# aitor-martinez-seras/SNN-Automotive-Object-Detection

Measured on AMD Instinct MI355X. Metric: images/sec (T_rpn=8,T_det=12, 1024x2048 b=2) spiking RPN+RoI heads forward, higher is better.
Workload: dtype f32 (weights as exact bf16x3 split, fp32 accumulate); 1 GPU; cityscapes_1024x2048_b2_heads: RPNHeadSNN(T=8) on 5-level pyramid 2x256x{192x384..12x24} + FastRCNNPredictorSNNFull(T=12) on 2000 RoIs x 12544, K=9; random-init weights; inputs: FPN output of the random-init ResNet-50-FPN on seeded rand(3,1024,2048) images (transform 768/1536); RoI features = 7x7 RoIAlign of 1000 seeded boxes per image; precision=bf16x3, global_batch=2, parallelism=dp1, exchange=none

## Files before the change

### snn_automotive_object_detection_amd/csrc/snn_kernels.hip

```cpp
#include "snn_common.h"
#include "snn_hip.h"
#include "snn_hip_debug.h"

#if !defined(SNN_EXPERIMENTS) && (defined(SNN_EXP_NO_FETCH) || defined(SNN_EXP_NO_GLDS) || defined(SNN_EXP_NO_BARRIER) || \
    defined(SNN_EXP_CLOCK) || defined(SNN_EXP_TIMELINE) || defined(SNN_EXP_SP_NO_A) || defined(SNN_EXP_SP_NO_B) || defined(SNN_EXP_SP_NO_AREAD) || defined(SNN_EXP_SP_NO_BREAD) || defined(SNN_EXP_SP_NO_MFMA) || defined(SNN_EXP_SP_NO_BAR) || defined(SNN_EXP_ONE_WG_PER_CU) || defined(SNN_EXP_MX_NOSTAGE) || defined(SNN_EXP_MX_NOREADB) || defined(SNN_EXP_MX_NOBAR) || \
    defined(SNN_EXP_MX_NOA) || defined(SNN_EXP_MX_BAR2) || defined(SNN_EXP_MX_RDW_G) || defined(SNN_EXP_ENCP_NOLOAD) || defined(SNN_EXP_ENCP_NOENC) || defined(SNN_EXP_ENCP_NOSTORE) || \
    defined(SNN_EXP_PP_NOWAIT) || defined(SNN_EXP_PP_NOCOPY) || defined(SNN_EXP_PP_NOBAR) || defined(SNN_EXP_PP_NOMFMA) || defined(SNN_EXP_PP_NOEPI) || defined(SNN_EXP_PP_NOY) || defined(SNN_EXP_PP_ALLDENSE) || defined(SNN_EXP_PP_ALLSPARSE) || defined(SNN_EXP_PP_NOBREAD) || defined(SNN_EXP_SP_NO_SEC))
#error "SNN_EXP_* switches are timing experiments with wrong results: add -DSNN_EXPERIMENTS (never in a product build)"
#endif

#include <stdarg.h>
#include <stdio.h>
#include <stdlib.h>
#include <string.h>

static thread_local char g_err[512] = "";
static thread_local int g_last_fc_sparse = 0;
static thread_local unsigned long long g_last_rpn_planes[3] = {0, 0, 0};
static thread_local unsigned long long g_last_det_planes[3] = {0, 0, 0};
static thread_local int g_last_enc_mode = -1;
static thread_local int g_last_conv_sparse = 0;

static int fail(int code, const char* fmt, ...) __attribute__((format(printf, 2, 3)));
static int fail(int code, const char* fmt, ...) {
// ... 85 lines not shown
        }
        dst[idx] = v;
    }
}

#include "snn_encode.h"
#include "snn_f32.h"
#include "snn_bf16x3.h"
#include "snn_sparse.h"
#ifdef SNN_PINGPONG
#include "snn_sparse_pp.h"
#endif
#include "snn_heads.h"
#include "snn_post.h"

#include "snn_mx.h"

#include "snn_affine.h"
#include "snn_taps.h"
#include "snn_wgrad.h"
#include "snn_loss.h"
#include "snn_hidden.h"
#include "snn_spike_wgrad_x3.h"

#define SNN_SPARSE_FAT_CONV_DEFAULT 3
#ifndef SNN_CONV_PP_DEFAULT
#define SNN_CONV_PP_DEFAULT 0
#endif
struct Knobs {
    bool enc_generic;
    bool enc_rows_ballot;
    int bf16x3_mt;
    int bf16x3_short;
    int bf16x3_wn;
    bool bf16x3_lif_reg;
    int mx_mw;
    int li_heads;
    bool debug_occ;
    bool spk_rows;
    bool bf16x3_xcd;
    bool stage_wm;
    bool enc_quant;
    bool periods;
    bool stage_periods;
    int roi_e, roi_rw;
    bool epi_general;
    bool roi_tab;
    bool dead_keep;
    bool sparse;
    int encp_nw;
    int encp_rb;
    int sparse_fat_conv;
    bool lif_regs;
    bool conv_pp;
    bool enc_fold;
    bool sparse_fat;
    int planes;
};
static Knobs load_knobs() {
    Knobs k;
    const char* e;
    k.enc_generic = (e = getenv("SNN_ENC_GENERIC")) && e[0] == '1';
    k.enc_rows_ballot = (e = getenv("SNN_ENC_ROWS")) && !strcmp(e, "ballot");
    k.bf16x3_mt = (e = getenv("SNN_BF16X3_MT")) ? atoi(e) : 0;
    e = getenv("SNN_BF16X3_SHORT");
    k.bf16x3_short = (e && e[0] == '1') ? 1 : (e && e[0] == '0') ? 0 : -1;
    e = getenv("SNN_BF16X3_WN");
    k.bf16x3_wn = (e && e[0] == '2') ? 2 : (e && e[0] == '1') ? 1 : 0;
    k.bf16x3_lif_reg = (e = getenv("SNN_BF16X3_LIF")) && !strcmp(e, "reg");
    e = getenv("SNN_MX_MW");
    k.mx_mw = (e && e[0] == '8') ? 8 : ((e && e[0] == '4') ? 4 : 0);
    e = getenv("SNN_LI_HEADS");
    k.li_heads = !e ? 0 : !strcmp(e, "valu") ? 1 : !strcmp(e, "mfma") ? 2 : !strcmp(e, "ksplit") ? 3 : 4;
    k.debug_occ = getenv("SNN_DEBUG_OCC") != nullptr;
    k.sparse_fat = !((e = getenv("SNN_SPARSE_FAT")) && e[0] == '0');
    k.enc_fold = !((e = getenv("SNN_ENC_FOLD")) && e[0] == '0');
    k.conv_pp = (e = getenv("SNN_CONV_PP")) ? e[0] == '1' : SNN_CONV_PP_DEFAULT != 0;
    k.lif_regs = !((e = getenv("SNN_LIF_REGS")) && e[0] == '0');
    k.sparse_fat_conv = (e = getenv("SNN_SPARSE_FAT_CONV")) ? atoi(e) : SNN_SPARSE_FAT_CONV_DEFAULT;
    k.encp_rb = (e = getenv("SNN_ENCP_RB")) ? atoi(e) : 0;
    k.encp_nw = (e = getenv("SNN_ENCP_NW")) ? atoi(e) : 0;
    e = getenv("SNN_PLANES");
    k.planes = !e ? 0 : !strcmp(e, "rm") ? 1 : !strcmp(e, "wm") ? 2 : 0;
    k.bf16x3_xcd = !((e = getenv("SNN_BF16X3_XCD")) && e[0] == '0');
    k.spk_rows = (e = getenv("SNN_SPK_SPLIT")) && e[0] == '0';
    k.stage_wm = (e = getenv("SNN_STAGE_PLANES")) && !strcmp(e, "wm");
    k.dead_keep = (e = getenv("SNN_DEAD_STEPS")) && !strcmp(e, "keep");
    k.periods = !((e = getenv("SNN_PERIOD_PLANES")) && e[0] == '0');
    k.enc_quant = !((e = getenv("SNN_ENC_QUANT")) && e[0] == '0');
    k.stage_periods = (e = getenv("SNN_STAGE_PERIODS")) && e[0] == '1';
    k.epi_general = (e = getenv("SNN_EPI_GENERAL")) && e[0] == '1';
    k.roi_tab = !((e = getenv("SNN_ROI_TAB")) && e[0] == '0');
    k.sparse = !((e = getenv("SNN_SPARSE")) && e[0] == '0');
    k.roi_e = (e = getenv("SNN_ROI_E")) ? atoi(e) : 0;
    k.roi_rw = (e = getenv("SNN_ROI_RW")) ? atoi(e) : 0;
    if (k.roi_e < 0 || k.roi_e > 16) k.roi_e = 0;
    if (k.roi_rw < 0 || k.roi_rw > 8) k.roi_rw = 0;
    return k;
}
// ... 92 lines not shown
    const int force = knobs().bf16x3_mt;
    if (force == 8 && knobs().bf16x3_wn == 2 && tiles_of(8) > 0) return 8;
    for (int mt = 4; mt >= 2; --mt) {
        const long long wgs = tiles_of(mt);
        if (wgs <= 0) continue;
        if (force == mt) return mt;
        const double cost = (double)((wgs + g3_slots() - 1) / g3_slots()) * (mt + 0.5);
        if (best_cost == 0 || cost < best_cost * 0.97) { best = mt; best_cost = cost; }
    }
    return best;
}

struct G3Tile { int mt, n_short, rows; };
template <typename F>
static G3Tile g3_pick_tile(int wn, F wgs_of) {
    G3Tile best = {0, 0, 0};
    double best_cost = 0;
    const int force_mt = knobs().bf16x3_mt, force_short = knobs().bf16x3_short;
    const int nwm = 8 / wn;
    if (force_mt == 8 && knobs().bf16x3_wn == 2 && wgs_of(256) > 0) return G3Tile{8, 0, 256};
    for (int mt = 4; mt >= 2; --mt)
        for (int sh = 0; sh < 2; ++sh) {
            if (force_mt >= 2 && force_mt <= 4 && force_mt != mt) continue;
            if (force_short >= 0 && force_short != sh) continue;
            const int n_short = sh ? nwm / 2 : 0, rows = nwm * 16 * mt - 16 * n_short;
            const long long wgs = wgs_of(rows);
            if (wgs <= 0) continue;
            const double cost = (double)((wgs + g3_slots() - 1) / g3_slots()) * (mt - 0.5 * sh + 0.5);
            if (best_cost == 0 || cost < best_cost * 0.97) { best = G3Tile{mt, n_short, rows}; best_cost = cost; }
        }
    return best;
}

#ifndef G3_NB1
#define G3_NB1 4
#endif
static int g3_wn(bool conv = false) { (void)conv; return knobs().bf16x3_wn ? knobs().bf16x3_wn : 1; }

static int g3_bm(int wn, int mt) { return mt == 8 ? 256 : G3_BM(wn, mt); }

template <int MODE>
static const void* g3_kernel(int mt, int wn, int planes) {
    if (planes == 1) {
        if (wn == 2)
            return mt == 8 ? (const void*)k_gemm_bf16<MODE, 3, 8, 2>
                 : mt == 4 ? (const void*)k_gemm_bf16<MODE, 3, 4, 2> : mt == 3 ? (const void*)k_gemm_bf16<MODE, 3, 3, 2>
                                                                                : (const void*)k_gemm_bf16<MODE, 3, 2, 2>;
        return mt == 4 ? (const void*)k_gemm_bf16<MODE, G3_NB1, 4, 1> : mt == 3 ? (const void*)k_gemm_bf16<MODE, G3_NB1, 3, 1>
                                                                                  : (const void*)k_gemm_bf16<MODE, G3_NB1, 2, 1>;
    }
    if (wn == 2)
        return mt == 8 ? (const void*)k_gemm_bf16x3<MODE, 3, 8, 2>
             : mt == 4 ? (const void*)k_gemm_bf16x3<MODE, 3, 4, 2> : mt == 3 ? (const void*)k_gemm_bf16x3<MODE, 3, 3, 2>
                                                                              : (const void*)k_gemm_bf16x3<MODE, 3, 2, 2>;
    return mt == 4 ? (const void*)k_gemm_bf16x3<MODE, G3_NB1, 4, 1> : mt == 3 ? (const void*)k_gemm_bf16x3<MODE, G3_NB1, 3, 1>
                                                                                : (const void*)k_gemm_bf16x3<MODE, G3_NB1, 2, 1>;
}

__device__ __forceinline__ unsigned long long det_payload_key(const float* __restrict__ l, int K, int r) {
    float m = l[0];
    for (int c = 1; c < K; ++c) m = fmaxf(m, l[c]);
    float sum = 0.0f, best = -1.0f;
    int lab = 1;
    for (int c = 0; c < K; ++c) {
        const float e = expf(l[c] - m);
        sum += e;
        if (c >= 1 && e > best) { best = e; lab = c; }
    }
    const float score = best / sum;
    return ((unsigned long long)__float_as_uint(score) << 32) | ((unsigned long long)(0xFFFFu - (unsigned)r) << 16) | (unsigned)lab;
}

template <int E>
__global__ __launch_bounds__(1024) void k_det_payload(const float* __restrict__ cls, const float* __restrict__ reg, int Rn,
                                                      int K, int max_det, int npad, float* __restrict__ payload,
                                                      int* __restrict__ counts) {
    extern __shared__ __attribute__((aligned(16))) unsigned char smem[];
    unsigned long long* const keys = reinterpret_cast<unsigned long long*>(smem);
    const int img = blockIdx.x, tid = threadIdx.x, nthr = blockDim.x;
    const size_t base = (size_t)img * Rn;
    if (E == 1) {
        unsigned long long key = tid < Rn ? det_payload_key(cls + (base + tid) * K, K, tid) : 0ull;
        for (int k = 2; k <= npad; k <<= 1)
            for (int j = k >> 1; j > 0; j >>= 1) {
                unsigned long long other;
                if (j < 64) {
                    other = __shfl_xor(key, j);
                } else {
                    __syncthreads();
                    keys[tid] = key;
                    __syncthreads();
                    other = keys[tid ^ j];
                }
                const bool desc = (tid & k) == 0, lower = (tid & j) == 0;
                const bool take_max = desc == lower;
                key = take_max ? (key > other ? key : other) : (key < other ? key : other);
            }
        __syncthreads();
        keys[tid] = key;
        __syncthreads();
    } else {
        for (int r = tid; r < npad; r += nthr) keys[r] = r < Rn ? det_payload_key(cls + (base + r) * K, K, r) : 0ull;
        __syncthreads();
        for (int k = 2; k <= npad; k <<= 1)
            for (int j = k >> 1; j > 0; j >>= 1) {
                for (int i = tid; i < npad; i += nthr) {
                    const int ixj = i ^ j;
                    if (ixj > i) {
                        const unsigned long long a = keys[i], b = keys[ixj];
                        if ((i & k) == 0 ? a < b : a > b) { keys[i] = b; keys[ixj] = a; }
                    }
                }
                __syncthreads();
            }
    }
    const int n = min(max_det, Rn);
    for (int t = tid; t < max_det; t += nthr) {
        float* out = payload + ((size_t)img * max_det + t) * 6;
        if (t < n) {
            const unsigned long long key = keys[t];
            const int r = 0xFFFF - (int)((key >> 16) & 0xFFFFu), lab = (int)(key & 0xFFFFu);
            const float* d = reg + (base + r) * 4 * K + 4 * lab;
            out[0] = d[0]; out[1] = d[1]; out[2] = d[2]; out[3] = d[3];
            out[4] = __uint_as_float((uint32_t)(key >> 32));
            out[5] = (float)lab;
        } else {
            for (int q = 0; q < 6; ++q) out[q] = 0.0f;
        }
    }
    if (tid == 0) counts[img] = n;
}

#define ENC_PICKER(fn, K, KN)                                                                                                                              \
    template <int EM>                                                                                                                                      \
    static const void* fn##_of(int fdt) {                                                                                                                  \
        if (fdt & SNN_FEAT_NHWC) return KN<EM>(fdt & ~SNN_FEAT_NHWC);                                                                                      \
        return fdt == SNN_FEAT_F16 ? (const void*)K##_h<EM, feat_f16> : fdt == SNN_FEAT_BF16 ? (const void*)K##_h<EM, feat_bf16> : (const void*)K<EM>;      \
    }                                                                                                                                                      \
    static const void* fn(int em, int fdt) { return em == ENC_QUANT ? fn##_of<ENC_QUANT>(fdt) : em == ENC_ZR ? fn##_of<ENC_ZR>(fdt) : fn##_of<ENC_GENERIC>(fdt); }
template <int EM> static const void* enc_nhwc_stage(int dt) {
    return dt == SNN_FEAT_F16 ? (const void*)k_encode_nhwc<EM, feat_f16> : dt == SNN_FEAT_BF16 ? (const void*)k_encode_nhwc<EM, feat_bf16> : (const void*)k_encode_nhwc<EM, float>;
}
template <int EM> static const void* enc_nhwc_levels(int dt) {
    return dt == SNN_FEAT_F16 ? (const void*)k_encode_levels_nhwc<EM, feat_f16> : dt == SNN_FEAT_BF16 ? (const void*)k_encode_levels_nhwc<EM, feat_bf16>
                                                                                                       : (const void*)k_encode_levels_nhwc<EM, float>;
}
template <int EM> static const void* enc_nhwc_none(int) { return nullptr; }
ENC_PICKER(encode_nchw_kernel, k_encode_nchw, enc_nhwc_stage)
ENC_PICKER(encode_levels_kernel, k_encode_levels, enc_nhwc_levels)
ENC_PICKER(encode_rows_wm_kernel, k_encode_rows_wm, enc_nhwc_none)
#undef ENC_PICKER
static size_t feat_elem_bytes(int fdt) { return (fdt & ~SNN_FEAT_NHWC) == SNN_FEAT_F32 ? 4 : 2; }
template <int RB, int NW>
// ... 269 lines not shown
                                  snn_stream_t s) {
    if (!a_rows || !w_packed || !cur || M <= 0 || K <= 0 || N <= 0 || ldo < N)
        return fail(-1, "snn_spike_gemm_bf16x3: bad argument");
    Gemm3Args a;
    memset(&a, 0, sizeof(a));
    if ((long long)M * cdiv(K, 32) * 4 > 0xffffffffLL) return fail(-1, "snn_spike_gemm_bf16x3: spike rows over 4 GB");
    a.A = a_rows; a.wpk = w_packed; a.out = cur; a.M = M; a.Kc = cdiv(K, 32); a.Np = cdiv(N, 32) * 32; a.ldo = ldo;
    a.plane_elems = (unsigned long long)a.Kc * a.Np * 32;
    const int wn = g3_wn();
    a.n_blocks = cdiv(a.Np, G3_BN(wn));
    const int mt = g3_pick_mt([&](int m) { return (long long)cdiv(M, g3_bm(wn, m)) * a.n_blocks; });
    return launch_gemm3(G3_FC, mt, wn, a, planes, (hipStream_t)s);
}

int snn_spike_gemm_bf16x3(const uint32_t* a_rows, int M, int K, int N, const uint16_t* w_packed, float* cur, int ldo,
                          snn_stream_t s) {
    return spike_gemm_bf16x3_impl(a_rows, M, K, N, w_packed, cur, ldo, 3, s);
}

static int set_periods(Gemm3Args& a, const char* who) {
    if (a.t0 != 0) return fail(-1, "%s: period planes need a window that starts at step 0", who);
    a.periods = 1;
    for (int t = 0; t < SNN_MAX_STEPS; ++t) {
        a.div[t] = 0;
        if (t < a.Tc)
            for (int n = 1; n <= a.Tc; ++n)
                if ((t + 1) % n == 0) a.div[t] |= 1u << (n - 1);
    }
    return 0;
}

static int spike_gemm_lif_bf16x3_args(const uint32_t* a_planes, int T, int R, int K, int N, const snn_params* p,
                                      const uint16_t* w_packed, uint32_t* spk, size_t spk_stride, uint32_t* row_counts,
                                      bool wm_in, bool wm_out, const StepWindow* win, bool periods, Gemm3Args* out, G3Tile* tile) {
    if (!a_planes || !w_packed || !spk || !p || R <= 0 || K <= 0 || N <= 0)
        return fail(-1, "snn_spike_gemm_lif_bf16x3: bad argument");
    if (check_T(T, "snn_spike_gemm_lif_bf16x3")) return -1;
    if ((long long)T * R * cdiv(K, 32) * 4 > 0xffffffffLL) return fail(-1, "snn_spike_gemm_lif_bf16x3: input planes over 4 GB");
    Gemm3Args& a = *out;
    memset(&a, 0, sizeof(a));
    a.A = a_planes; a.wpk = w_packed; a.M = R; a.Kc = cdiv(K, 32); a.Np = cdiv(N, 32) * 32;
    a.plane_elems = (unsigned long long)a.Kc * a.Np * 32;
    const int wn = g3_wn();
    a.n_blocks = cdiv(a.Np, G3_BN(wn));
    a.T = T; a.spk = spk; a.spk_stride = spk_stride; a.p = make_p(p, p->v_th_lif); a.cnt_row = row_counts;
    a.wm = wm_in; a.out_wm = wm_out; a.a_step = (unsigned long long)R;
    const StepWindow w = win ? *win : lif_window_full_out(T);
    a.t0 = w.t0; a.Tc = w.n;
    const int Tc = w.n;
    const G3Tile tl = g3_pick_tile(wn, [&](int rows) { return g3_tile_ok(Tc, rows) ? (long long)cdiv(R, rows / Tc) * a.n_blocks : 0ll; });
    if (!tl.mt) return fail(-4, "snn_spike_gemm_lif_bf16x3: T=%d does not fit a row tile (use snn_spike_gemm_bf16x3 + snn_lif_scan)", T);
    a.pb = tl.rows / Tc; a.n_short = tl.n_short;
    if (periods && set_periods(a, "snn_spike_gemm_lif_bf16x3")) return -1;
    *tile = tl;
    return 0;
}

static int spike_gemm_lif_bf16x3_impl(const uint32_t* a_planes, int T, int R, int K, int N, const snn_params* p,
                                      const uint16_t* w_packed, uint32_t* spk, size_t spk_stride, uint32_t* row_counts, snn_stream_t s,
                                      bool wm_in = false, bool wm_out = false, const StepWindow* win = nullptr, bool periods = false) {
    Gemm3Args a;
    G3Tile tl;
    const int rc = spike_gemm_lif_bf16x3_args(a_planes, T, R, K, N, p, w_packed, spk, spk_stride, row_counts, wm_in, wm_out, win, periods, &a, &tl);
    if (rc) return rc;
    return launch_gemm3(G3_FC_LIF_TILE, tl.mt, g3_wn(), a, 3, (hipStream_t)s);
}

int snn_spike_gemm_lif_bf16x3(const uint32_t* a_planes, int T, int R, int K, int N, const snn_params* p,
                              const uint16_t* w_packed, uint32_t* spk, size_t spk_stride, snn_stream_t s) {
    return spike_gemm_lif_bf16x3_impl(a_planes, T, R, K, N, p, w_packed, spk, spk_stride, nullptr, s, knobs().stage_wm, false, nullptr,
                                      knobs().stage_periods);
}

static bool mx_tile_ok(int T) { return g3_tile_ok(T, MX_BM); }

static int mx_mw() { return knobs().mx_mw ? knobs().mx_mw : MX_MW_DEFAULT; }

#define MX_KERNEL_OF(MW, mode)                                                                        \
    ((mode) == G3_FC ? (const void*)k_gemm_mx<G3_FC, MW>                                              \
     : (mode) == G3_CONV ? (const void*)k_gemm_mx<G3_CONV, MW>                                        \
     : (mode) == G3_CONV_LIF_TILE ? (const void*)k_gemm_mx<G3_CONV_LIF_TILE, MW>                      \
                                  : (const void*)k_gemm_mx<G3_FC_LIF_TILE, MW>)

// ... 360 lines not shown
    SNN_CHECK_LAUNCH("k_gemm_lif_sparse");
    }
    if (cnt_pos) {
        PosCountArgs pa;
        memset(&pa, 0, sizeof(pa));
        pa.cnt_pos = cnt_pos; pa.cnt_img = a.cnt_img; pa.n_levels = a.n_levels; pa.max_n = a.max_n;
        memcpy(pa.lv, a.lv, sizeof(pa.lv));
        hipLaunchKernelGGL(k_sum_pos_counts, dim3(a.n_levels * a.max_n, POSCNT_CHUNKS), dim3(256), 0, s, pa);
        SNN_CHECK_LAUNCH("k_sum_pos_counts");
    }
    return gated ? 2 : 1;
}

int snn_debug_tile_shape(int conv, long long units, int k_in, int n_cols, int num_steps, int spike_rates, int layer, int32_t* out) {
    if (!out || units <= 0 || k_in <= 0 || n_cols <= 0 || num_steps < 1 || num_steps > SNN_MAX_STEPS) return fail(-1, "snn_debug_tile_shape: bad argument");
    snn_params p;
    memset(&p, 0, sizeof(p));
    p.v_th_lif = 0.1f;
    int Tc;
    if (conv) Tc = lif_window_full_out(num_steps).n;
    else { const DetWindows w = det_windows(&p, num_steps, spike_rates != 0); Tc = layer == 7 ? w.fc7.n : w.fc6.n; }
    memset(out, 0, 12 * sizeof(int32_t));
    SparseShape sh;
    const int Kw = cdiv(k_in, 32), Np = cdiv(n_cols, 32) * 32;
    if (knobs().periods && (conv || layer != 7) && sparse_shape(conv != 0, units, Kw, conv ? 9 * Kw : Kw, Np, num_steps, Tc, SPARSE_ROUTE, &sh)) {
        const SparsePlan& sp = sh.sp;
        int slots = 0;
        for (int w = 0; w < (sp.fat ? 4 : 8) / sp.wn; ++w) slots += sp.w_nd[w] + sp.w_ns[w];
        out[0] = sp.fat ? (sp.wn == 1 ? SP_MT_FAT : conv ? SP_MT2_FAT_CONV : SP_MT2_FAT) : sp.wn == 1 ? SP_MT : SP_MT2; out[1] = sp.fat; out[2] = Tc * sp.pb; out[3] = sp.pb; out[4] = Tc; out[5] = sh.n_tiles * sh.n_blocks;
        out[6] = sh.n_blocks; out[7] = sp.wn; out[8] = 1; out[9] = sp.nd; out[10] = Tc - sp.nd; out[11] = slots;
        return 0;
    }
    const int wn = g3_wn(conv != 0), n_blocks = cdiv(Np, G3_BN(wn));
    const G3Tile tl = g3_pick_tile(wn, [&](int rows) { return g3_tile_ok(Tc, rows) ? (long long)cdiv(units, rows / Tc) * n_blocks : 0ll; });
    if (!tl.mt) return fail(-4, "snn_debug_tile_shape: %d steps do not fit a row tile", num_steps);
    const int pb = tl.rows / Tc;
    out[0] = tl.mt; out[1] = tl.n_short; out[2] = tl.rows; out[3] = pb; out[4] = Tc; out[5] = (int32_t)(cdiv(units, pb) * n_blocks);
    out[6] = n_blocks; out[7] = wn; out[8] = 0; out[9] = Tc; out[10] = 0; out[11] = 0;
    return 0;
}

struct ConvLifOpts {
    bool wm = false;
    bool* out_split = nullptr;
    bool periods = false;
    void* sparse_side = nullptr;
    size_t sparse_bytes = 0;
    int sparse_mode = SPARSE_RUN;
    SparseRoute route = SPARSE_ROUTE;
    int planes = 3;
};
static int conv3x3_lif_bf16x3_impl(const uint32_t* enc, size_t enc_stride, const snn_rpn_level* lv, int n_levels, int C_in,
                                   int C_out, int T, const snn_params* p, const uint16_t* w_packed, uint32_t* spk,
                                   size_t spk_stride, unsigned long long* counts, int max_n, snn_stream_t s, const ConvLifOpts& o) {
    const bool wm = o.wm, periods = o.periods;
    const int sparse_mode = o.sparse_mode;
    const bool want_split = o.out_split && *o.out_split;
    if (o.out_split) *o.out_split = false;
    if (!spk || !p) return fail(-1, "snn_conv3x3_lif_bf16x3: bad argument");
    Gemm3Args a;
    long long P;
    int rc = conv3_common("snn_conv3x3_lif_bf16x3", enc, enc_stride, lv, n_levels, C_in, C_out, T, w_packed, a, &P);
    if (rc) return rc;
    if (wm) {
        if (enc_stride % a.Cw) return fail(-1, "snn_conv3x3_lif_bf16x3: word-major planes need enc_stride %% Cw == 0");
        a.wm = 1; a.a_step = enc_stride / a.Cw;
        if (a.a_step * (unsigned long long)a.Cw > 0x7fffffffULL) return fail(-1, "snn_conv3x3_lif_bf16x3: plane too large");
// ... 1164 lines not shown
static DetCall det_call(int fdt, int R, int Hd, int K, int K4, int T, const snn_params* p, const void* w6_packed, int w6_inner,
                        const void* w7_packed, const float* w_heads_packed, float* out_cls, float* out_bbox, uint32_t* spk6_count,
                        uint32_t* spk7_count, float* sum_cls, float* sum_bbox, void* ws, size_t ws_bytes, snn_stream_t stream) {
    DetCall c = {};
    c.fdt = fdt; c.R = R; c.Hd = Hd; c.K = K; c.K4 = K4; c.T = T; c.p = p;
    c.w6_packed = w6_packed; c.w6_inner = w6_inner; c.w7_packed = w7_packed; c.w_heads_packed = w_heads_packed;
    c.out_cls = out_cls; c.out_bbox = out_bbox; c.spk6_count = spk6_count; c.spk7_count = spk7_count; c.sum_cls = sum_cls; c.sum_bbox = sum_bbox;
    c.ws = ws; c.ws_bytes = ws_bytes; c.stream = stream;
    c.route = SPARSE_ROUTE;
    return c;
}
static void feed_rows(DetCall& c, const void* x, int D) { c.roi_fed = false; c.x = x; c.D = D; c.who = "snn_det_head_forward"; }
static void feed_roialign(DetCall& c, const snn_roi_level* levels_host, int n_levels, int C, const float* rois, const int* roi_batch,
                          const int* roi_level) {
    c.roi_fed = true; c.levels_host = levels_host; c.n_levels = n_levels; c.C = C; c.rois = rois; c.roi_batch = roi_batch; c.roi_level = roi_level;
    c.who = "snn_det_head_forward_roialign";
}

static int det_readouts_check(const char* who, const int* steps, int n, const uint32_t* c6, const uint32_t* c7, const float* sum_cls,
                              const float* sum_bbox) {
    if (check_steps(steps, n, who)) return -1;
    if ((c6 == nullptr) != (c7 == nullptr)) return fail(-1, "%s: spk6_count and spk7_count go together", who);
    if ((sum_cls == nullptr) != (sum_bbox == nullptr)) return fail(-1, "%s: sum_cls and sum_bbox go together", who);
    return 0;
}

struct DetPlan {
    size_t o_enc, o_cur, o_s6, o_s7;
    size_t o_raw;
    DetWindows win;
    bool wm, per;
    bool bin_major;
    bool gated;
};

static void det_planes_views(const DetPlan& dp, int R, int Hd, int T, snn_planes_view* v6, snn_planes_view* v7) {
    const int Hw = cdiv(Hd, 32);
    for (int i = 0; i < 2; ++i) {
        snn_planes_view* v = i ? v7 : v6;
        if (!v) continue;
        const StepWindow& w = i ? dp.win.fc7 : dp.win.fc6;
        v->offset_bytes = i ? dp.o_s7 : dp.o_s6; v->step_stride_words = (uint64_t)R * Hw; v->rows = R; v->words = Hw;
        v->layout = (!i && dp.wm) ? SNN_PLANES_WORD_MAJOR : SNN_PLANES_ROWS;
        v->steps_formed = min(T, w.t0 + w.n + 1);
        v->reserved = 0;
    }
}

static bool det_fc6_sparse_plan(const DetCall& c, int D, const DetPlan& dp) {
    Gemm3Args a6;
    G3Tile t6;
    return spike_gemm_lif_bf16x3_args((const uint32_t*)((char*)c.ws + dp.o_enc), c.T, c.R, D, c.Hd, c.p, (const uint16_t*)c.w6_packed,
                                      (uint32_t*)((char*)c.ws + dp.o_s6), (size_t)c.R * cdiv(c.Hd, 32), c.spk6_count, true, true, &dp.win.fc6, true,
                                      &a6, &t6) == 0 &&
           gemm3_lif_sparse(a6, false, (char*)c.ws + dp.o_cur, dp.o_s6 - dp.o_cur, (hipStream_t)c.stream, SPARSE_QUERY, c.route, weight_planes(c.p)) == 1;
}

static int det_plan(const DetCall& c, int D, bool wm_ok, DetPlan* dp) {
    size_t need;
    det_ws_layout(c.R, D, c.Hd, c.T, &dp->o_enc, &dp->o_cur, &dp->o_s6, &dp->o_s7, &need);
    if (c.ws_bytes < need) return fail(-2, "%s: workspace %zu < %zu bytes", c.who, c.ws_bytes, need);
    if (check_T(c.T, c.who)) return -1;
    dp->o_raw = c.w6_inner > 1 ? det_ws_perm_offset(c.R, D, c.Hd, c.T) : dp->o_enc;
    dp->bin_major = false;
    dp->win = det_windows(c.p, c.T, c.spk6_count != nullptr);
    dp->wm = det_planes_wm(c.p, dp->win) && wm_ok;
    dp->per = knobs().periods && periods_possible(c.p) && det_b3_tiles(c.p, dp->win);
    dp->gated = c.route.route == SNN_ROUTE_AUTO && c.route.stat && !c.spk6_count && !c.steps && c.w6_inner == 49 && dp->wm && dp->per &&
                det_fc6_sparse_plan(c, D, *dp);
    return 0;
}

static bool det_fc6_folds(bool feed_ok, const DetCall& c, int D, const DetPlan& dp, NeuronP* np, const EncTh** eth) {
    if (dp.gated || !knobs().enc_fold || !feed_ok || c.w6_inner != 49 || !dp.wm || !dp.per) return false;
    *np = make_p(c.p, c.p->v_th_enc);
    np->v_fire = ENC_FIRED;
    if (!enc_zero_rest(*np) || enc_mode(*np, eth) != ENC_QUANT) return false;
    return det_fc6_sparse_plan(c, D, dp);
}

static int det_heads_tail(const DetCall& c, const uint32_t* s6, const uint32_t* s7, bool s6_wm) {
    const int R = c.R, Hw = cdiv(c.Hd, 32);
    if (!c.steps)
        return snn_li_heads(s7, (size_t)R * Hw, c.T, R, c.Hd, c.w_heads_packed, c.K, c.K4, c.p, c.out_cls, c.out_bbox, c.sum_cls, c.sum_bbox, c.stream);
    int rc = li_heads_readouts_impl(s7, (size_t)R * Hw, c.steps, c.n_steps, R, c.Hd, c.w_heads_packed, c.K, c.K4, c.p, c.out_cls, c.out_bbox, c.sum_cls,
                                    c.sum_bbox, false, c.stream);
    if (rc || !c.spk6_count) return rc;
    const StepList st = step_list(c.steps, c.n_steps);
    hipLaunchKernelGGL(k_count_rows_ro, dim3(cdiv(R, 256)), dim3(256), 0, (hipStream_t)c.stream, s6, (unsigned long long)R * Hw, R, Hw, s6_wm ? 1 : 0, st, c.spk6_count);
    SNN_CHECK_LAUNCH("k_count_rows_ro");
    hipLaunchKernelGGL(k_count_rows_ro, dim3(cdiv(R, 256)), dim3(256), 0, (hipStream_t)c.stream, s7, (unsigned long long)R * Hw, R, Hw, 0, st, c.spk7_count);
    SNN_CHECK_LAUNCH("k_count_rows_ro");
    return 0;
}

static int fc6_route_fixed(int32_t* route_stat, int route_taken, hipStream_t s) {
    if (!route_stat) return 0;
// ... 22 lines not shown
    const int Hw = cdiv(Hd, 32), Hp = Hw * 32;
    snn_planes_view v6, v7;
    det_planes_views(dp, R, Hd, T, &v6, &v7);
    g_last_det_planes[0] = v6.offset_bytes; g_last_det_planes[1] = v7.offset_bytes; g_last_det_planes[2] = v6.layout == SNN_PLANES_WORD_MAJOR ? 1 : 0;
    int rc;
    if (k_inner > 1 && !folded && !dp.bin_major) {
        const int C = D / k_inner;
        if (D % k_inner || C % 32 || !enc_wm || !det_b3_tiles(p, win))
            return fail(-4, "snn_det_head_forward: permuted fc6 weights (inner = %d) need D = C * inner, C %% 32 == 0 and the fused bf16x3 path", k_inner);
        const uint32_t* enc_raw = (const uint32_t*)((char*)ws + dp.o_raw);
        const int Dw = cdiv(D, 32);
        if (k_inner != 49) return fail(-4, "snn_det_head_forward: permuted fc6 weights: inner = %d (only 49 = 7 x 7 bins is built)", k_inner);
        hipLaunchKernelGGL(k_permute_planes<49>, dim3(cdiv(R, 32), win.enc_steps), dim3(256), 0, s, enc_raw, enc, Dw, R, C);
        SNN_CHECK_LAUNCH("k_permute_planes");
    }
    if (spk6_count) { if (hipMemsetAsync(spk6_count, 0, sizeof(uint32_t) * R, s) != hipSuccess) return fail(-3, "hipMemsetAsync failed"); }
    if (spk7_count) { if (hipMemsetAsync(spk7_count, 0, sizeof(uint32_t) * R, s) != hipSuccess) return fail(-3, "hipMemsetAsync failed"); }
    const bool b3 = prec_family(p) == SNN_PRECISION_BF16X3, mx = prec_family(p) == SNN_PRECISION_MXFP6;
    if (prec_family(p) != SNN_PRECISION_F32 && !b3 && !mx) return fail(-1, "snn_det_head_forward: unknown precision %d", p->precision);
    if (mx) {
        if (D % 128 || Hd % 128)
            return fail(-4, "snn_det_head_forward: the mxfp6 kernels need D, Hd %% 128 == 0");
        if (!mx_tile_ok(win.fc6.n) || !mx_tile_ok(win.fc7.n)) return fail(-4, "snn_det_head_forward: T=%d does not fit a 512-row tile of the mxfp6 kernels", T);
        if ((rc = fc6_route_fixed(rt.stat, spk6_count ? 0 : 1, s))) return rc;
        if ((rc = spike_gemm_lif_mx_impl(enc, T, R, D, Hd, p, (const uint32_t*)w6_packed, s6, (size_t)R * Hw, spk6_count, stream, &win.fc6))) return rc;
        if ((rc = spike_gemm_lif_mx_impl(s6, T, R, Hd, Hd, p, (const uint32_t*)w7_packed, s7, (size_t)R * Hw, spk7_count, stream, &win.fc7))) return rc;
        return det_heads_tail(c, s6, s7, false);
    }
    if ((enc_wm || enc_periods) && !det_b3_tiles(p, win)) return fail(-1, "snn_det_head_forward: word-major / period planes without the fused bf16x3 layers");
    if (det_b3_tiles(p, win)) {
        Gemm3Args a6, a7;
        G3Tile t6, t7;
        if ((rc = spike_gemm_lif_bf16x3_args(enc, T, R, D, Hd, p, (const uint16_t*)w6_packed, s6, (size_t)R * Hw, spk6_count, enc_wm, enc_wm, &win.fc6, enc_periods, &a6, &t6))) return rc;
        if ((rc = spike_gemm_lif_bf16x3_args(s6, T, R, Hd, Hd, p, (const uint16_t*)w7_packed, s7, (size_t)R * Hw, spk7_count, enc_wm, false, &win.fc7, false, &a7, &t7))) return rc;
        const int wn = g3_wn();
        rc = gemm3_lif_sparse(a6, false, (char*)ws + o_cur, o_s6 - o_cur, s, folded ? SPARSE_RUN_COMPRESSED : SPARSE_RUN, rt, planes);
        if (rc < 0) return rc;
        if (folded && rc != 1) return fail(-3, "snn_det_head_forward: the encoder wrote compressed planes but fc6 takes the dense launch (internal)");
        if (rt.gated && rc != 2) return fail(-3, "snn_det_head_forward: fc6 route: the gated pair was planned but fc6 did not enqueue it (internal)");
        g_last_fc_sparse = rc;
        if (rc == 2) { a6.gate = (const int*)rt.stat + 2; a6.gate_want = 1; }
        else if ((rc = fc6_route_fixed(rt.stat, (spk6_count || rc == 1) ? 0 : 1, s))) return rc;
        if (g_last_fc_sparse != 1 && (rc = launch_gemm3(G3_FC_LIF_TILE, t6.mt, wn, a6, planes, s))) return rc;
        if ((rc = launch_gemm3(G3_FC_LIF_TILE, t7.mt, wn, a7, planes, s))) return rc;
        return det_heads_tail(c, s6, s7, enc_wm);
    }
    if ((rc = fc6_route_fixed(rt.stat, spk6_count ? 0 : 1, s))) return rc;
    const uint32_t* a6 = enc + (size_t)win.fc6.t0 * R * cdiv(D, 32);
    rc = b3 ? spike_gemm_bf16x3_impl(a6, win.fc6.n * R, D, Hd, (const uint16_t*)w6_packed, cur, Hp, planes, stream)
            : snn_spike_gemm(a6, win.fc6.n * R, D, Hd, (const float*)w6_packed, cur, Hp, stream);
    if (rc) return rc;
    if ((rc = lif_scan_window(cur, T, win.fc6, R, Hd, Hp, p, s6, (size_t)R * Hw, spk6_count, stream))) return rc;
    const uint32_t* a7 = s6 + (size_t)win.fc7.t0 * R * Hw;
    rc = b3 ? spike_gemm_bf16x3_impl(a7, win.fc7.n * R, Hd, Hd, (const uint16_t*)w7_packed, cur, Hp, planes, stream)
            : snn_spike_gemm(a7, win.fc7.n * R, Hd, Hd, (const float*)w7_packed, cur, Hp, stream);
    if (rc) return rc;
    if ((rc = lif_scan_window(cur, T, win.fc7, R, Hd, Hp, p, s7, (size_t)R * Hw, spk7_count, stream))) return rc;
    return det_heads_tail(c, s6, s7, false);
}

static int det_encode_rows(const DetCall& c, const DetPlan& dp, bool* folded) {
    const void* const x = c.x;
    const int R = c.R, D = c.D;
    if (c.w6_inner > 1 && !dp.wm) return fail(-4, "snn_det_head_forward: permuted fc6 weights need the word-major fused bf16x3 path (D %% 32 == 0, x 16-byte aligned)");
    NeuronP np;
    const EncTh* eth_f = nullptr;
    const bool fold = *folded = det_fc6_folds(D % (49 * 64) == 0, c, D, dp, &np, &eth_f);
// ... 200 lines not shown
                                int32_t* route_stat, snn_stream_t stream) {
    const size_t need = p ? snn_det_head_workspace_bytes_routed(R, D, Hd, K, K4, T, p->precision, route) : 0;
    if (route_check("snn_det_head_forward_routed", route, crossover, route_stat, ws_bytes, need)) return -1;
    DetCall c = det_call(fdt, R, Hd, K, K4, T, p, w6_packed, w6_inner, w7_packed, w_heads_packed, out_cls, out_bbox, spk6_count, spk7_count, sum_cls,
                         sum_bbox, ws, ws_bytes, stream);
    feed_rows(c, x, D);
    c.route = routed(route, crossover, route_stat, spk6_count != nullptr);
    return det_head_run(c);
}

int snn_det_head_forward_roialign_routed(const snn_roi_level* levels_host, int fdt, int n_levels, int C, const float* rois,
                                         const int* roi_batch, const int* roi_level, int R, int Hd, int K, int K4, int T,
                                         const snn_params* p, const void* w6_packed, int w6_inner, const void* w7_packed,
                                         const float* w_heads_packed, float* out_cls, float* out_bbox, uint32_t* spk6_count,
                                         uint32_t* spk7_count, float* sum_cls, float* sum_bbox, void* ws, size_t ws_bytes,
                                         int route, float crossover, int32_t* route_stat, snn_stream_t stream) {
    const size_t need = p ? snn_det_head_workspace_bytes_routed(R, C > 0 && C < (1 << 24) ? C * 49 : 0, Hd, K, K4, T, p->precision, route) : 0;
    if (route_check("snn_det_head_forward_roialign_routed", route, crossover, route_stat, ws_bytes, need)) return -1;
    DetCall c = det_call(fdt, R, Hd, K, K4, T, p, w6_packed, w6_inner, w7_packed, w_heads_packed, out_cls, out_bbox, spk6_count, spk7_count, sum_cls,
                         sum_bbox, ws, ws_bytes, stream);
    feed_roialign(c, levels_host, n_levels, C, rois, roi_batch, roi_level);
    c.route = routed(route, crossover, route_stat, spk6_count != nullptr);
    return det_head_run(c);
}

int snn_det_exchange_payload(const float* class_logits, const float* box_regression, int N, int rois_per_image, int K,
                             int max_det, float* payload, int* counts, snn_stream_t s) {
    if (!class_logits || !box_regression || !payload || !counts || N <= 0 || rois_per_image <= 0 || K < 2 || max_det <= 0)
        return fail(-1, "snn_det_exchange_payload: bad argument");
    if (rois_per_image > 4096 || K > 0xFFFF) return fail(-4, "snn_det_exchange_payload: %d RoIs per image (max 4096)", rois_per_image);
    int npad = 64;
    while (npad < rois_per_image) npad <<= 1;
    if (npad <= 1024)
        hipLaunchKernelGGL(k_det_payload<1>, dim3(N), dim3(npad), (size_t)npad * 8, (hipStream_t)s, class_logits,
                           box_regression, rois_per_image, K, max_det, npad, payload, counts);
    else
        hipLaunchKernelGGL(k_det_payload<4>, dim3(N), dim3(1024), (size_t)npad * 8, (hipStream_t)s, class_logits,
                           box_regression, rois_per_image, K, max_det, npad, payload, counts);
    SNN_CHECK_LAUNCH("k_det_payload");
    return 0;
}

static_assert(SNN_PLANES_ROWS == TAP_LAYOUT_ROWS && SNN_PLANES_SPLIT4 == TAP_LAYOUT_SPLIT4 && SNN_PLANES_WORD_MAJOR == TAP_LAYOUT_WORD_MAJOR,
              "snn_taps.h addresses the layouts of include/snn_hip.h");

int snn_rpn_head_planes_view(const snn_rpn_level* lv, int n_levels, int C, int A, int T, const snn_params* p, int route, int spike_rates,
                             snn_planes_view* shared_lif) {
    (void)spike_rates;
    if (!lv || !p || !shared_lif) return fail(-1, "snn_rpn_head_planes_view: null argument");
    if (n_levels <= 0 || n_levels > SNN_MAX_LEVELS || C <= 0 || A <= 0) return fail(-1, "snn_rpn_head_planes_view: bad n_levels / C / A");
    if (!route_known(route)) return fail(-1, "snn_rpn_head_planes_view: unknown route %d", route);
    if (prec_family(p) != SNN_PRECISION_F32 && prec_family(p) != SNN_PRECISION_BF16X3 && prec_family(p) != SNN_PRECISION_MXFP6)
        return fail(-1, "snn_rpn_head_planes_view: unknown precision %d", p->precision);
    if (check_T(T, "snn_rpn_head_planes_view")) return -1;
    for (int l = 0; l < n_levels; ++l)
        if (lv[l].N <= 0 || lv[l].H <= 0 || lv[l].W <= 0) return fail(-1, "snn_rpn_head_planes_view: bad level %d", l);
    const long long P = rpn_positions(lv, n_levels, nullptr);
    size_t o_spk, o_cur, o_cnt, need;
    rpn_ws_layout(P, prec_family(p) != SNN_PRECISION_F32 ? rpn_positions_padded(lv, n_levels) : 0, C, T, prec_family(p), &o_spk, &o_cur, &o_cnt, &need);
    rpn_planes_view(p, P, C, A, T, o_spk, shared_lif);
    return 0;
}

int snn_det_head_planes_view(int R, int D, int Hd, int K, int K4, int T, const snn_params* p, int w6_inner, int route, int spike_rates,
                             snn_planes_view* lif6, snn_planes_view* lif7) {
    if (!p || (!lif6 && !lif7)) return fail(-1, "snn_det_head_planes_view: null argument");
    if (R <= 0 || D <= 0 || Hd <= 0 || K <= 0 || K4 <= 0) return fail(-1, "snn_det_head_planes_view: bad shape");
// ... 376 lines not shown
```

Before: 765.1 images/s.

## Replace bitonic sort in detection payload with radix top-k select and rank scatter

For the single-wave-per-RoI path of the detection payload kernel, when max_det is at most 128, a byte-wise radix select over the 64-bit score keys first finds the top-n threshold. Only the selected keys are then sorted, by counting how many selected keys exceed each one, in place of a full bitonic sort over all padded keys. The launch reserves extra shared memory for the histogram and state. A separate SNN_FC7_ROWS environment knob can force the fc7 row tile, but it is off by default.

```diff
diff --git a/snn_automotive_object_detection_amd/csrc/snn_kernels.hip b/snn_automotive_object_detection_amd/csrc/snn_kernels.hip
--- a/snn_automotive_object_detection_amd/csrc/snn_kernels.hip
+++ b/snn_automotive_object_detection_amd/csrc/snn_kernels.hip
@@ -141,6 +141,7 @@
     bool enc_rows_ballot;
     int bf16x3_mt;
     int bf16x3_short;
+    int fc7_rows;
     int bf16x3_wn;
     bool bf16x3_lif_reg;
     int mx_mw;
@@ -174,6 +175,7 @@
     k.bf16x3_mt = (e = getenv("SNN_BF16X3_MT")) ? atoi(e) : 0;
     e = getenv("SNN_BF16X3_SHORT");
     k.bf16x3_short = (e && e[0] == '1') ? 1 : (e && e[0] == '0') ? 0 : -1;
+    k.fc7_rows = (e = getenv("SNN_FC7_ROWS")) ? atoi(e) : 0;
     e = getenv("SNN_BF16X3_WN");
     k.bf16x3_wn = (e && e[0] == '2') ? 2 : (e && e[0] == '1') ? 1 : 0;
     k.bf16x3_lif_reg = (e = getenv("SNN_BF16X3_LIF")) && !strcmp(e, "reg");
@@ -332,6 +334,16 @@
     return best;
 }
 
+static G3Tile g3_tile_of_rows(int wn, int want_rows) {
+    const int nwm = 8 / wn;
+    for (int mt = 4; mt >= 2; --mt)
+        for (int sh = 0; sh < 2; ++sh) {
+            const int n_short = sh ? nwm / 2 : 0, rows = nwm * 16 * mt - 16 * n_short;
+            if (rows == want_rows) return G3Tile{mt, n_short, rows};
+        }
+    return G3Tile{0, 0, 0};
+}
+
 #ifndef G3_NB1
 #define G3_NB1 4
 #endif
@@ -379,7 +391,64 @@
     unsigned long long* const keys = reinterpret_cast<unsigned long long*>(smem);
     const int img = blockIdx.x, tid = threadIdx.x, nthr = blockDim.x;
     const size_t base = (size_t)img * Rn;
-    if (E == 1) {
+    const unsigned long long* sorted = keys;
+    if (E == 1 && npad > 128 && min(max_det, Rn) <= 128) {
+        unsigned int* const hist = reinterpret_cast<unsigned int*>(keys + npad);
+        unsigned int* const st = hist + 256;
+        const int n = min(max_det, Rn);
+        const unsigned long long key = tid < Rn ? det_payload_key(cls + (base + tid) * K, K, tid) : 0ull;
+        for (int i = tid; i < 256 + 4; i += nthr) hist[i] = 0u;
+        __syncthreads();
+        bool tied = tid < Rn, taken = false;
+        unsigned int need = (unsigned int)n;
+        for (int shift = 56; shift >= 0; shift -= 8) {
+            const unsigned int byte = (unsigned int)(key >> shift) & 0xFFu;
+            if (tied) atomicAdd(&hist[byte], 1u);
+            __syncthreads();
+            if (tid < 64) {
+                unsigned int c[4], s = 0u;
+                for (int q = 0; q < 4; ++q) { c[q] = hist[4 * tid + q]; hist[4 * tid + q] = 0u; s += c[q]; }
+                unsigned int v = s;
+                for (int d = 1; d < 64; d <<= 1) {
+                    const unsigned int o = __shfl_down(v, d);
+                    if (tid + d < 64) v += o;
+                }
+                unsigned int above = v - s;
+                for (int q = 3; q >= 0; --q) {
+                    if (above < need && need <= above + c[q]) { st[0] = 4u * tid + q; st[1] = need - above; st[2] = c[q]; }
+                    above += c[q];
+                }
+            }
+            __syncthreads();
+            const unsigned int bin = st[0], in_bin = st[2];
+            need = st[1];
+            if (tied && byte != bin) { tied = false; taken = byte > bin; }
+            if (in_bin == need) break;
+        }
+        taken = taken || tied;
+        const unsigned long long m = __ballot(taken);
+        const int lane = tid & 63;
+        unsigned int slot = 0u;
+        if (lane == 0 && m) slot = atomicAdd(&st[3], (unsigned int)__popcll(m));
+        slot = __shfl(slot, 0) + (unsigned int)__popcll(m & ((1ull << lane) - 1ull));
+        if (taken) keys[slot] = key;
+        if (tid == n && (n & 1)) keys[n] = 0ull;
+        __syncthreads();
+        unsigned long long* const by_rank = keys + npad / 2;
+        if (tid < n) {
+            const unsigned long long mine = keys[tid];
+            const ulonglong2* const pairs = reinterpret_cast<const ulonglong2*>(keys);
+            int rank = 0;
+#pragma unroll 4
+            for (int j = 0; j < (n + 1) / 2; ++j) {
+                const ulonglong2 v = pairs[j];
+                rank += (v.x > mine ? 1 : 0) + (v.y > mine ? 1 : 0);
+            }
+            by_rank[rank] = mine;
+        }
+        __syncthreads();
+        sorted = by_rank;
+    } else if (E == 1) {
         unsigned long long key = tid < Rn ? det_payload_key(cls + (base + tid) * K, K, tid) : 0ull;
         for (int k = 2; k <= npad; k <<= 1)
             for (int j = k >> 1; j > 0; j >>= 1) {
@@ -418,7 +487,7 @@
     for (int t = tid; t < max_det; t += nthr) {
         float* out = payload + ((size_t)img * max_det + t) * 6;
         if (t < n) {
-            const unsigned long long key = keys[t];
+            const unsigned long long key = sorted[t];
             const int r = 0xFFFF - (int)((key >> 16) & 0xFFFFu), lab = (int)(key & 0xFFFFu);
             const float* d = reg + (base + r) * 4 * K + 4 * lab;
             out[0] = d[0]; out[1] = d[1]; out[2] = d[2]; out[3] = d[3];
@@ -754,7 +823,8 @@
 
 static int spike_gemm_lif_bf16x3_args(const uint32_t* a_planes, int T, int R, int K, int N, const snn_params* p,
                                       const uint16_t* w_packed, uint32_t* spk, size_t spk_stride, uint32_t* row_counts,
-                                      bool wm_in, bool wm_out, const StepWindow* win, bool periods, Gemm3Args* out, G3Tile* tile) {
+                                      bool wm_in, bool wm_out, const StepWindow* win, bool periods, Gemm3Args* out, G3Tile* tile,
+                                      int force_rows = 0) {
     if (!a_planes || !w_packed || !spk || !p || R <= 0 || K <= 0 || N <= 0)
         return fail(-1, "snn_spike_gemm_lif_bf16x3: bad argument");
     if (check_T(T, "snn_spike_gemm_lif_bf16x3")) return -1;
@@ -770,7 +840,11 @@
     const StepWindow w = win ? *win : lif_window_full_out(T);
     a.t0 = w.t0; a.Tc = w.n;
     const int Tc = w.n;
-    const G3Tile tl = g3_pick_tile(wn, [&](int rows) { return g3_tile_ok(Tc, rows) ? (long long)cdiv(R, rows / Tc) * a.n_blocks : 0ll; });
+    G3Tile tl = g3_pick_tile(wn, [&](int rows) { return g3_tile_ok(Tc, rows) ? (long long)cdiv(R, rows / Tc) * a.n_blocks : 0ll; });
+    if (force_rows > 0) {
+        tl = g3_tile_of_rows(wn, force_rows);
+        if (!tl.mt || !g3_tile_ok(Tc, tl.rows)) return fail(-4, "snn_spike_gemm_lif_bf16x3: no row tile of %d rows for %d time steps (SNN_FC7_ROWS)", force_rows, Tc);
+    }
     if (!tl.mt) return fail(-4, "snn_spike_gemm_lif_bf16x3: T=%d does not fit a row tile (use snn_spike_gemm_bf16x3 + snn_lif_scan)", T);
     a.pb = tl.rows / Tc; a.n_short = tl.n_short;
     if (periods && set_periods(a, "snn_spike_gemm_lif_bf16x3")) return -1;
@@ -1197,7 +1271,11 @@
         return 0;
     }
     const int wn = g3_wn(conv != 0), n_blocks = cdiv(Np, G3_BN(wn));
-    const G3Tile tl = g3_pick_tile(wn, [&](int rows) { return g3_tile_ok(Tc, rows) ? (long long)cdiv(units, rows / Tc) * n_blocks : 0ll; });
+    G3Tile tl = g3_pick_tile(wn, [&](int rows) { return g3_tile_ok(Tc, rows) ? (long long)cdiv(units, rows / Tc) * n_blocks : 0ll; });
+    if (!conv && layer == 7 && knobs().fc7_rows > 0) {
+        tl = g3_tile_of_rows(wn, knobs().fc7_rows);
+        if (tl.mt && !g3_tile_ok(Tc, tl.rows)) tl.mt = 0;
+    }
     if (!tl.mt) return fail(-4, "snn_debug_tile_shape: %d steps do not fit a row tile", num_steps);
     const int pb = tl.rows / Tc;
     out[0] = tl.mt; out[1] = tl.n_short; out[2] = tl.rows; out[3] = pb; out[4] = Tc; out[5] = (int32_t)(cdiv(units, pb) * n_blocks);
@@ -2428,6 +2506,7 @@
     bool wm, per;
     bool bin_major;
     bool gated;
+    int fc7_rows;
 };
 
 static void det_planes_views(const DetPlan& dp, int R, int Hd, int T, snn_planes_view* v6, snn_planes_view* v7) {
@@ -2459,6 +2538,7 @@
     if (check_T(c.T, c.who)) return -1;
     dp->o_raw = c.w6_inner > 1 ? det_ws_perm_offset(c.R, D, c.Hd, c.T) : dp->o_enc;
     dp->bin_major = false;
+    dp->fc7_rows = knobs().fc7_rows;
     dp->win = det_windows(c.p, c.T, c.spk6_count != nullptr);
     dp->wm = det_planes_wm(c.p, dp->win) && wm_ok;
     dp->per = knobs().periods && periods_possible(c.p) && det_b3_tiles(c.p, dp->win);
@@ -2547,7 +2627,7 @@
         Gemm3Args a6, a7;
         G3Tile t6, t7;
         if ((rc = spike_gemm_lif_bf16x3_args(enc, T, R, D, Hd, p, (const uint16_t*)w6_packed, s6, (size_t)R * Hw, spk6_count, enc_wm, enc_wm, &win.fc6, enc_periods, &a6, &t6))) return rc;
-        if ((rc = spike_gemm_lif_bf16x3_args(s6, T, R, Hd, Hd, p, (const uint16_t*)w7_packed, s7, (size_t)R * Hw, spk7_count, enc_wm, false, &win.fc7, false, &a7, &t7))) return rc;
+        if ((rc = spike_gemm_lif_bf16x3_args(s6, T, R, Hd, Hd, p, (const uint16_t*)w7_packed, s7, (size_t)R * Hw, spk7_count, enc_wm, false, &win.fc7, false, &a7, &t7, dp.fc7_rows))) return rc;
         const int wn = g3_wn();
         rc = gemm3_lif_sparse(a6, false, (char*)ws + o_cur, o_s6 - o_cur, s, folded ? SPARSE_RUN_COMPRESSED : SPARSE_RUN, rt, planes);
         if (rc < 0) return rc;
@@ -2814,7 +2894,7 @@
     int npad = 64;
     while (npad < rois_per_image) npad <<= 1;
     if (npad <= 1024)
-        hipLaunchKernelGGL(k_det_payload<1>, dim3(N), dim3(npad), (size_t)npad * 8, (hipStream_t)s, class_logits,
+        hipLaunchKernelGGL(k_det_payload<1>, dim3(N), dim3(npad), (size_t)npad * 8 + (256 + 4) * 4, (hipStream_t)s, class_logits,
                            box_regression, rois_per_image, K, max_det, npad, payload, counts);
     else
         hipLaunchKernelGGL(k_det_payload<4>, dim3(N), dim3(1024), (size_t)npad * 8, (hipStream_t)s, class_logits,
```

Result: no change. 767.6 images/s, median of 6 (+0.3%).
